# chenghuige/golden-huffman

Hardware: AMD Instinct MI355X
Metric: encode+decode GB/s (input bytes) (higher is better)
Workload: dtype u8

## Files before the change

golden-huffman_amd/csrc/ghf_internal.h:

```cpp
#ifndef GHF_INTERNAL_H_
#define GHF_INTERNAL_H_
#include <hip/hip_runtime.h>
#include <stdint.h>
#include <type_traits>
#include "ghf.h"

namespace ghf {

constexpr int kWave = 64;
constexpr int kSymPerLane = 16;
constexpr int kSymPerIter = kWave * kSymPerLane;
constexpr int kSegSymbols = 64;
constexpr int kBlockSymbols = 4096;
constexpr uint32_t kChunkQuantum = 4096;
constexpr uint32_t kMinChunk = 16384;
constexpr uint32_t kMaxChunk = 1u << 20;
constexpr uint32_t kEmitSlots = 256 * 3 * 8;

constexpr int kHistThreads = 256;
constexpr int kHistRep = 32;

constexpr int kEmitThreads = 512;
constexpr int kEmitWaves = kEmitThreads / kWave;
constexpr int kStageWords = 544;
constexpr int kStageCapBits = (kStageWords - 8) * 32;

constexpr int kDecPairBitsMax = 10;
constexpr int kDecLutBitsMax = 12;
constexpr int kDec7LutLog2 = 14;
constexpr int kDec7LutSlots = 1 << kDec7LutLog2;
constexpr int kDec7SmallSlots = 1024;

constexpr uint32_t kPlanesGroups = 256 * 16;
constexpr uint32_t kPlanesLdsBytes = 9 * 1024;
__host__ __device__ constexpr inline uint32_t planes_tile_elems(uint32_t elem_bytes) {
  return (uint32_t)kWave * (elem_bytes < 4 ? 4 : elem_bytes) * 16 / elem_bytes;
}
template <class F>
inline void with_elem_bytes(uint32_t elem_bytes, F&& f) {
  if (elem_bytes == 2) f(std::integral_constant<int, 2>());
  else if (elem_bytes == 4) f(std::integral_constant<int, 4>());
  else f(std::integral_constant<int, 8>());
}
constexpr int kPlanesHistThreads = 256;
constexpr int kPlanesHistCols = 32;
constexpr uint32_t kPlanesHistGroups = 256 * 4;
constexpr uint32_t kPlanesHistTileVecs = kPlanesHistThreads * 4;
constexpr uint32_t kPlanesHistFlushTiles = 3;
static_assert((uint64_t)(kPlanesHistFlushTiles + 1) * kPlanesHistTileVecs * 16 < (1ull << 32), "a u32 counter never wraps between two flushes");
constexpr size_t kPlanesHistAccWords = 32 * GHF_PLANES_MAX * 256;
constexpr uint32_t kSparseTile = 4096;
constexpr uint32_t kSparseGroups = 256 * 16;
constexpr uint32_t kSparseLdsBytes = 258 * 16;
constexpr size_t kSparseOffWords = kSparseGroups + 2;
constexpr uint32_t kSparseRankElems = 32768;
constexpr size_t kSparseRankHeaderBytes = 64;
constexpr uint64_t kSparseRankMagic = 0x314B4E4152464847ull;
constexpr uint32_t kSparseRankVersion = 1;
static_assert(kSparseRankElems == 8 * kBlockSymbols, "a rank block of the mask is one seek block");

constexpr uint64_t kHeaderFixedBytes = 4 * (GHF_NSYM + 3);
template <class T>
__host__ __device__ constexpr inline T header_bytes_for(T max_len) { return (T)kHeaderFixedBytes + 8 * max_len; }
__host__ __device__ constexpr inline uint64_t blocks_for(uint64_t n) { return (n + kBlockSymbols - 1) / kBlockSymbols; }
__host__ __device__ constexpr inline uint64_t segs_for(uint64_t n) { return (n + kSegSymbols - 1) / kSegSymbols; }
inline void index_shape(uint64_t n, ghf_index* ix) {
  ix->n_symbols = n;
  ix->chunk_symbols = kBlockSymbols;
  ix->seg_symbols = kSegSymbols;
  ix->n_chunks = blocks_for(n);
  ix->n_segs = segs_for(n);
}

inline uint32_t chunk_symbols_for(uint64_t n) {
  const uint64_t per_slot = (n + kEmitSlots - 1) / kEmitSlots;
  uint64_t c = (per_slot + kChunkQuantum - 1) / kChunkQuantum * kChunkQuantum;
  if (c < kMinChunk) c = kMinChunk;
  if (c > kMaxChunk) c = kMaxChunk;
  return (uint32_t)c;
}
inline uint64_t chunk_count_for(uint64_t n) {
  const uint64_t c = chunk_symbols_for(n);
  return (n + c - 1) / c;
}

struct DecTables {
  uint32_t fc_left[36];
  uint32_t start_pos[36];
  uint16_t symbol[GHF_NSYM + 3];
  int32_t min_len, max_len, lut_bits;
  int32_t pair_bits;
  int32_t kind;
  uint32_t root;
  uint16_t tl[256], tr[256];
  uint32_t ticket[16 * 32];
  uint32_t done;
  alignas(16) uint32_t image[kDec7LutSlots + kDec7SmallSlots];
};

struct EmitParams {
  const uint8_t* in;
  uint64_t n;
  const ghf_code* code;
  const uint64_t* chunk_off;
  const uint64_t* d_start_bit;
  uint8_t* out;
  uint64_t cap;
  uint32_t chunk;
  uint32_t nchunks;
  uint64_t* chunk_bit;
  uint32_t* seg_bit;
  int flags;
  int* status;
  uint64_t* d_end;
};

struct DecParams {
  const uint8_t* stream;
  uint64_t stream_bytes;
  DecTables* dt;
  const uint64_t* chunk_bit;
  const uint32_t* seg_bit;
  uint64_t n_symbols;
  uint64_t n_segs;
  uint32_t no_end_mark;
  uint8_t* out;
  uint64_t* out_bytes;
  int* status;
};

constexpr int kRunSymbols = 512;
constexpr int kRunsPerBlock = kBlockSymbols / kRunSymbols;
constexpr int kRunSegs = kRunSymbols / kSegSymbols;
constexpr size_t kSeekHeaderBytes = 64;
constexpr size_t kSeekRecordBytes = 24;
constexpr uint64_t kSeekMagic = 0x314B454553464847ull;
constexpr uint32_t kSeekVersion = 1;

struct SeekPackParams {
  const uint64_t* chunk_bit;
  const uint32_t* seg_bit;
  uint64_t n_symbols, n_blocks, n_segs;
  uint32_t flags;
  uint8_t* table;
  int* status;
};
struct SeekExpandParams {
  const uint8_t* records;
  const uint8_t* stream;
  uint64_t stream_bytes;
  const DecTables* dt;
  uint64_t n_symbols, n_blocks;
  uint64_t g0, g1;
  uint64_t* chunk_bit;
  uint32_t* seg_bit;
  int* status;
};
struct SeekExpandPlanesParams {
  SeekExpandParams plane[GHF_PLANES_MAX];
};
constexpr uint32_t kSeekStreamsMax = 2 * GHF_PLANES_MAX;
struct SeekExpandStreamsParams {
  SeekExpandParams stream[kSeekStreamsMax];
};
static_assert(sizeof(SeekExpandStreamsParams) <= 4096 - 64, "the parameter block stays under the kernel-argument limit");
struct DecHeadParams {
  const uint8_t* stream;
  uint64_t stream_bytes;
  const DecTables* dt;
  const uint64_t* chunk_bit;
  const uint32_t* seg_bit;
  uint64_t blk_sym0;
  uint64_t n_symbols;
  uint64_t lo, hi;
  uint8_t* out;
  int* status;
};

struct BatchCompressParams {
  const uint8_t* const* in_ptrs;
  const uint64_t* in_bytes;
  uint64_t max_item_bytes;
  uint8_t* const* out_ptrs;
  const uint64_t* out_caps;
  uint64_t* out_bytes;
  ghf_code* codes;
  uint64_t* chunk_bit;
  uint32_t* seg_bit;
  uint64_t blocks_per_item, segs_per_item;
  int* item_status;
};
struct BatchDecodeParams {
  const uint8_t* const* stream_ptrs;
  const uint64_t* stream_bytes;
  const ghf_code* codes;
  const uint64_t* chunk_bit;
  const uint32_t* seg_bit;
  uint64_t blocks_per_item, segs_per_item;
  uint64_t max_item_bytes;
  const uint64_t* n_symbols;
  uint8_t* const* out_ptrs;
  const uint64_t* out_caps;
  uint64_t* out_bytes;
  int* item_status;
};
struct BatchImagesParams {
  const uint8_t* const* stream_ptrs;
  const uint64_t* stream_bytes;
  uint64_t max_stream_bytes;
  uint8_t* const* out_ptrs;
  const uint64_t* out_caps;
  uint64_t* out_bytes;
  ghf_code* codes;
  int* item_status;
  uint64_t* stats;
};

struct BatchHistParams {
  const uint8_t* const* in_ptrs;
  const uint64_t* in_bytes;
  uint64_t max_item_bytes;
  uint32_t count;
  uint64_t* hist;
};
struct BatchSharedCompressParams {
  const uint8_t* const* in_ptrs;
  const uint64_t* in_bytes;
  uint64_t max_item_bytes;
  const ghf_code* code;
  uint8_t* const* out_ptrs;
  const uint64_t* out_caps;
  uint64_t* out_bytes;
  uint64_t* chunk_bit;
  uint32_t* seg_bit;
  uint64_t blocks_per_item, segs_per_item;
  int* item_status;
};
struct BatchSharedDecodeParams {
  const uint8_t* const* stream_ptrs;
  const uint64_t* stream_bytes;
  const ghf_code* code;
  const uint64_t* chunk_bit;
  const uint32_t* seg_bit;
  uint64_t blocks_per_item, segs_per_item;
  uint64_t max_item_bytes;
  const uint64_t* n_symbols;
  uint8_t* const* out_ptrs;
  const uint64_t* out_caps;
  uint64_t* out_bytes;
  int* item_status;
};
struct BatchSharedBodiesParams {
  const uint8_t* const* stream_ptrs;
  const uint64_t* stream_bytes;
  uint64_t max_stream_bytes;
  const ghf_code* code;
  uint8_t* const* out_ptrs;
  const uint64_t* out_caps;
  uint64_t* out_bytes;
  int* item_status;
  uint64_t* stats;
};

struct BatchPlanesHistParams {
  const uint8_t* const* in_ptrs;
  const uint64_t* in_bytes;
  uint64_t max_item_bytes;
  uint32_t count;
  uint64_t* hists;
};
struct BatchPlanesCompressParams {
  const uint8_t* const* in_ptrs;
  const uint64_t* in_bytes;
  uint64_t max_item_bytes;
  const ghf_code* codes;
  uint8_t* const* out_ptrs;
  const uint64_t* out_caps;
  uint64_t* out_bytes;
  uint64_t* chunk_bit;
  uint32_t* seg_bit;
  uint64_t blocks_per_item, segs_per_item;
  int* item_status;
};
struct BatchPlanesDecodeParams {
  const uint8_t* const* stream_ptrs;
  const uint64_t* stream_bytes;
  const ghf_code* codes;
  const uint64_t* chunk_bit;
  const uint32_t* seg_bit;
  uint64_t blocks_per_item, segs_per_item;
  uint64_t max_plane_symbols;
  const uint64_t* n_elems;
  uint8_t* const* out_ptrs;
  const uint64_t* out_caps;
  uint64_t* out_bytes;
  int* item_status;
};
struct BatchPlanesBodiesParams {
  const uint8_t* const* stream_ptrs;
  const uint64_t* stream_bytes;
  uint64_t max_stream_bytes;
  const ghf_code* codes;
  uint8_t* const* out_ptrs;
  const uint64_t* out_caps;
  uint64_t* out_bytes;
  int* item_status;
  uint64_t* stats;
};

constexpr uint32_t kBatchSeekMagic = 0x31524247u;
constexpr uint32_t kBatchRunSymbols = 128;
constexpr uint32_t kBatchRunSegs = kBatchRunSymbols / kSegSymbols;
constexpr uint32_t kBatchRunsPerBlock = kBlockSymbols / kBatchRunSymbols;
constexpr uint32_t kBatchSeekHeadBytes = 8;
__host__ __device__ constexpr inline uint64_t batch_runs_for(uint64_t n) { return (n + kBatchRunSymbols - 1) / kBatchRunSymbols; }
__host__ __device__ constexpr inline uint64_t batch_seek_bytes_for(uint64_t n) {
  return (kBatchSeekHeadBytes + 2 * batch_runs_for(n) + 7) & ~7ull;
}
struct BatchSeekPackParams {
  const uint64_t* chunk_bit;
  const uint32_t* seg_bit;
  uint64_t blocks_per_item, segs_per_item;
  uint64_t max_slice_symbols;
  const uint64_t* in_bytes;
  uint32_t elem_bytes;
  uint8_t* const* rec_ptrs;
  const uint64_t* rec_caps;
  uint64_t* rec_bytes;
  int* slot_status;
};
struct BatchSeekDecodeParams {
  const uint8_t* const* stream_ptrs;
  const uint64_t* stream_bytes;
  const uint8_t* const* rec_ptrs;
  const uint64_t* rec_bytes;
  uint64_t max_stream_bytes;
  const ghf_code* codes;
  uint8_t* const* out_ptrs;
  const uint64_t* out_caps;
  uint64_t* out_bytes;
  int* item_status;
};

enum SyncKind : uint32_t {
  kSyncCrs2 = 0,
  kSyncCrs = 1,
  kSyncPiece = 2,
};
struct SyncParams {
  const uint8_t* stream;
  uint64_t stream_bytes;
  uint64_t body_bit0;
  uint64_t end_bit;
  uint32_t no_eof;
  const DecTables* dt;
  uint64_t nsub;
  uint16_t* start;
  uint16_t* used;
  uint32_t* cnt;
  uint8_t* eof;
  uint32_t first;
  uint32_t first_start;
  uint32_t* changed;
  unsigned long long* moved_first_inv;
  uint64_t* eof_sub;
  uint64_t* tile_sum;
};

constexpr size_t kHistAccWords = 32 * 256 + 16 + 16 * 16;
void launch_histogram(const uint8_t* d_in, uint64_t n, uint32_t chunk, uint32_t nchunks, uint32_t* d_chunk_hist,
                      uint64_t* d_hist, uint64_t* d_acc, bool add, hipStream_t s);
void launch_build_code(const uint64_t* d_hist, ghf_code* d_code, int* d_status, uint32_t flags, hipStream_t s);
void launch_write_header(const ghf_code* d_code, uint8_t* d_out, uint64_t cap, int* d_status, hipStream_t s);
void launch_plan(const uint8_t* d_in, uint64_t n, uint32_t chunk, uint32_t nchunks, const uint32_t* d_chunk_hist,
                 const ghf_code* d_code, uint64_t* d_chunk_off, uint64_t* d_total_bits, hipStream_t s);
void launch_scan(uint64_t* d_v, uint32_t count, uint64_t* d_total, hipStream_t s);
void launch_crs_build_code(const uint64_t* d_hist, ghf_tree* d_tree, ghf_code* d_code, uint64_t* d_start_bit, int* d_status,
                           hipStream_t s);
void launch_crs_finish(const ghf_tree* d_tree, const uint64_t* d_total_bits, uint8_t* d_out, uint64_t* d_out_bytes, int* d_status,
                       hipStream_t s);
void launch_stream_copy(const uint8_t* d_src, uint8_t* d_dst, uint64_t n, bool nt, hipStream_t s);
void launch_store_u64(uint64_t* d_dst, const uint64_t* d_src_opt, uint64_t add, hipStream_t s);
void launch_load_u16(uint64_t* d_dst, const uint16_t* d_src, hipStream_t s);
void launch_shard_start(const ghf_code* d_code, const uint64_t* d_totals, int rank, uint64_t* d_start_bit, hipStream_t s);
void launch_emit(const EmitParams& p, hipStream_t s);
void launch_build_decode_tables(const ghf_code* d_code, DecTables* d_dt, int* d_status, hipStream_t s);
void launch_build_decode_tables_slots(const ghf_code* d_codes, DecTables* d_dts, uint32_t count, uint32_t slots, int* d_status, hipStream_t s);
void launch_crs_decode_tables(const ghf_tree* d_tree, DecTables* d_dt, int* d_status, hipStream_t s);
constexpr uint64_t kDecMaxGroups = 0xFFFF0000ull;
void launch_decode(const DecParams& p, hipStream_t s);
void launch_sync_pass(const SyncParams& p, hipStream_t s);
void launch_sync_counts(const SyncParams& p, uint64_t* d_total, hipStream_t s);
size_t sync_scan_workspace(uint64_t nsub);
void launch_sync_scan(const SyncParams& p, uint8_t* ws, uint32_t stride ,
                      uint32_t entry , hipStream_t s);
void launch_sync_index(const SyncParams& p, uint64_t* d_seg_abs, uint64_t n_symbols, uint64_t* d_chunk_bit, uint32_t* d_seg_bit,
                       hipStream_t s);
void launch_seek_pack(const SeekPackParams& p, hipStream_t s);
void launch_seek_expand(const SeekExpandParams& p, hipStream_t s);
void launch_seek_expand_planes(const SeekExpandPlanesParams& a, uint32_t planes, hipStream_t s);
void launch_seek_expand_streams(const SeekExpandStreamsParams& a, uint32_t streams, hipStream_t s);
void launch_decode_head(const DecHeadParams& p, hipStream_t s);
void launch_compress_batch(const BatchCompressParams& p, uint32_t count, hipStream_t s);
void launch_decode_batch(const BatchDecodeParams& p, uint32_t count, hipStream_t s);
void launch_decode_images_batch(const BatchImagesParams& p, uint32_t count, hipStream_t s);
void launch_histogram_batch(const BatchHistParams& p, uint32_t flags, hipStream_t s);
void launch_compress_batch_shared(const BatchSharedCompressParams& p, uint32_t count, hipStream_t s);
void launch_decode_batch_shared(const BatchSharedDecodeParams& p, uint32_t count, hipStream_t s);
void launch_decode_bodies_batch_shared(const BatchSharedBodiesParams& p, uint32_t count, hipStream_t s);
void launch_histogram_batch_finish(uint64_t* d_hists, uint32_t n_hists, uint32_t flags, hipStream_t s);
void launch_histogram_batch_planes(const BatchPlanesHistParams& p, uint32_t elem_bytes, uint32_t flags, hipStream_t s);
void launch_build_codes(const uint64_t* d_hists, uint32_t n_codes, ghf_code* d_codes, int* d_status, uint32_t flags, hipStream_t s);
void launch_batch_planes_raw_auto(const uint64_t* d_hists, const ghf_code* d_codes, uint32_t elem_bytes, uint32_t* d_raw_planes,
                                  hipStream_t s);
void launch_compress_batch_planes(const BatchPlanesCompressParams& p, uint32_t count, uint32_t elem_bytes, bool forms, uint32_t raw_planes,
                                  hipStream_t s);
void launch_decode_batch_planes(const BatchPlanesDecodeParams& p, uint32_t count, uint32_t elem_bytes, bool forms, uint32_t raw_planes,
                                hipStream_t s);
void launch_decode_bodies_batch_planes(const BatchPlanesBodiesParams& p, uint32_t count, uint32_t elem_bytes, bool forms,
                                       uint32_t raw_planes, hipStream_t s);
void launch_batch_seek_pack(const BatchSeekPackParams& p, uint32_t slots, hipStream_t s);
void launch_decode_bodies_batch_seek(const BatchSeekDecodeParams& p, uint32_t count, uint32_t elem_bytes, bool forms, uint32_t raw_planes,
                                     hipStream_t s);
void launch_planes_split(const uint8_t* d_in, const uint8_t* d_base, uint64_t n_elems, uint32_t elem_bytes, uint8_t* d_planes,
                         uint64_t plane_stride, hipStream_t s);
void launch_planes_merge(const uint8_t* d_planes, uint64_t plane_stride, const uint8_t* d_base, uint64_t n_elems, uint32_t elem_bytes,
                         uint8_t* d_out, const int* d_status, hipStream_t s);
void launch_planes_merge_range(const uint8_t* d_planes, uint64_t plane_stride, const uint8_t* d_base, uint64_t first, uint64_t count,
                               uint32_t elem_bytes, uint8_t* d_out, const int* d_status, hipStream_t s);
void launch_planes_split_to(const uint8_t* d_in, const uint8_t* d_base, uint64_t n_elems, uint32_t elem_bytes, uint8_t* const* h_dst,
                            hipStream_t s);
void launch_planes_merge_from(const uint8_t* const* h_src, const uint8_t* d_base, uint64_t n_elems, uint32_t elem_bytes, uint8_t* d_out,
                              const int* d_status, hipStream_t s);
void launch_sparse_split(const uint8_t* d_in, uint64_t n, uint8_t* d_mask, uint8_t* d_vals, uint64_t vals_cap, uint64_t* d_n_vals,
                         uint64_t* d_counts, uint64_t* d_offs, int* d_status, hipStream_t s);
void launch_sparse_merge(const uint8_t* d_mask, const uint8_t* d_vals, uint64_t n_vals, uint64_t n, uint8_t* d_out, uint64_t* d_counts,
                         uint64_t* d_offs, int* d_status, hipStream_t s);
void launch_sparse_merge_at(const uint8_t* d_mask, const uint8_t* d_vals, uint64_t vals_skip, uint64_t n_vals, uint64_t n, uint8_t* d_out,
                            uint64_t* d_counts, uint64_t* d_offs, int* d_status, hipStream_t s);
void launch_sparse_rank_pack(const uint8_t* d_mask, uint64_t n, uint8_t* d_table, uint64_t* d_counts, uint64_t* d_offs, int* d_status,
                             hipStream_t s);
hipError_t launch_histogram_planes(const uint8_t* d_in, const uint8_t* d_base, uint64_t n_elems, uint32_t elem_bytes, uint32_t flags,
                                   uint64_t* d_acc, uint64_t* d_hists, hipStream_t s);
void launch_planes_image_bytes(const uint64_t* d_hists, const ghf_code* d_codes, uint32_t elem_bytes, uint64_t* d_bytes, hipStream_t s);
void launch_planes_vet_codes(const uint64_t* d_hists, const ghf_code* d_codes, uint32_t elem_bytes, int* d_status, hipStream_t s);

struct PlanesGatherParams {
  const uint8_t* streams[GHF_PLANES_MAX];
  uint64_t stream_bytes[GHF_PLANES_MAX];
  const uint8_t* records[GHF_PLANES_MAX];
  const ghf_code* codes;
  uint64_t n_elems, n_blocks;
  const uint64_t* index;
  uint64_t index_stride;
  uint32_t row_elems, n_rows;
  uint32_t stage_bytes;
  uint8_t* out;
  uint64_t out_stride;
  int32_t* row_status;
};
void launch_decode_planes_gather(const PlanesGatherParams& p, uint32_t elem_bytes, uint32_t raw_planes, hipStream_t s);

struct PlanesGatherFormsParams {
  const uint8_t* streams[2 * GHF_PLANES_MAX];
  uint64_t stream_bytes[2 * GHF_PLANES_MAX];
  const uint8_t* records[2 * GHF_PLANES_MAX];
  const uint64_t* cum[GHF_PLANES_MAX];
  uint64_t n_vals[GHF_PLANES_MAX];
  const ghf_code* codes;
  const uint8_t* base;
  uint64_t n_elems;
  const uint64_t* index;
  uint64_t index_stride;
  uint32_t row_elems, n_rows;
  uint32_t stage_bytes;
  uint32_t once;
  uint8_t* out;
  uint64_t out_stride;
  int32_t* row_status;
};
void launch_decode_planes_gather_forms(const PlanesGatherFormsParams& p, uint32_t elem_bytes, uint32_t raw_planes, uint32_t sparse_planes,
                                       hipStream_t s);

}
#endif
```

golden-huffman_amd/csrc/ghf_kernels.hip:

```cpp
#include "ghf_build_code.h"

namespace ghf {

#define GHF_HADD(x, sh) atomicAdd(&lh[((((x) >> (sh)) & 0xFFu) << 5) | rep], 1u)

__device__ __forceinline__ void hist_vec(uint32_t* lh, uint32_t rep, const uint4& v) {
  GHF_HADD(v.x, 0); GHF_HADD(v.x, 8); GHF_HADD(v.x, 16); GHF_HADD(v.x, 24);
  GHF_HADD(v.y, 0); GHF_HADD(v.y, 8); GHF_HADD(v.y, 16); GHF_HADD(v.y, 24);
  GHF_HADD(v.z, 0); GHF_HADD(v.z, 8); GHF_HADD(v.z, 16); GHF_HADD(v.z, 24);
  GHF_HADD(v.w, 0); GHF_HADD(v.w, 8); GHF_HADD(v.w, 16); GHF_HADD(v.w, 24);
}

__global__ __launch_bounds__(kHistThreads) void k_histogram(const uint8_t* __restrict__ in, uint64_t n,
                                                            uint32_t chunk32, uint32_t nchunks,
                                                            uint32_t* __restrict__ chunk_hist,
                                                            unsigned long long* __restrict__ hist,
                                                            unsigned long long* __restrict__ acc ,
                                                            uint32_t add ) {
  static_assert(kHistRep == 32, "replica index is lane % 32");
  __shared__ uint32_t lh[256 * kHistRep];
  __shared__ bool s_last;
  const uint32_t tid = threadIdx.x;
  const uint32_t rep = tid & 31u;
  uint32_t prev = 0;
  unsigned long long total = 0;
  const uint64_t chunk = chunk32;
  const uint32_t V = chunk32 >> 12;
  const uint32_t nfullchunks = (uint32_t)(n / chunk);
  const bool fast = V >= 4u && (chunk32 & 4095u) == 0 && (((uintptr_t)in) & 15u) == 0 && nfullchunks > 0;
  auto vptr = [&](uint32_t c, uint32_t j) -> const uint4* {
    if (c >= nfullchunks) c = nfullchunks - 1;
    return reinterpret_cast<const uint4*>(in + (uint64_t)c * chunk) + (uint64_t)j * kHistThreads + tid;
  };
  uint4 A = make_uint4(0, 0, 0, 0), B = A;
  if (fast) {
    A = load_stream(vptr(blockIdx.x, 0));
    B = load_stream(vptr(blockIdx.x, 1));
  }
  for (uint32_t i = tid; i < 256 * kHistRep; i += kHistThreads) lh[i] = 0;
  __syncthreads();

  __shared__ uint32_t s_tick;
  auto finish_chunk = [&](uint32_t c) -> uint32_t {
    __syncthreads();
    const uint32_t posted = s_tick;
    uint32_t s = 0;
#pragma unroll
    for (uint32_t j = 0; j < kHistRep; ++j) s += lh[(tid << 5) | ((j + tid) & 31u)];
    const uint32_t cnt = s - prev;
    prev = s;
    chunk_hist[(uint64_t)c * 256 + tid] = cnt;
    total += cnt;
    __syncthreads();
    return posted;
  };

  if (fast) {
    const uint32_t ncls = gridDim.x < 16u ? 1u : (gridDim.x < 128u ? gridDim.x >> 3 : 16u);
    const uint32_t cls = (blockIdx.x >> 3) % ncls;
    unsigned long long* tick = acc + 32 * 256 + 16 + cls * 16;
    auto draw = [&]() -> uint32_t { return 2u * gridDim.x + (uint32_t)atomicAdd(tick, 1ull) * ncls + cls; };
    uint32_t cur = blockIdx.x;
    uint32_t nxt = blockIdx.x + gridDim.x;
    auto vat = [&](uint32_t g) -> const uint4* { return g < V ? vptr(cur, g) : vptr(nxt, g - V); };
    const uint32_t Vmain = V & ~3u, Vrest = V & 3u;
    while (cur < nfullchunks) {
      uint32_t t_next = 0;
      if (tid == 0) t_next = draw();
      for (uint32_t j = 0; j < Vmain; j += 4) {
        const uint4 C = load_stream(vat(j + 2)), D = load_stream(vat(j + 3));
        hist_vec(lh, rep, A);
        hist_vec(lh, rep, B);
        A = load_stream(vat(j + 4));
        B = load_stream(vat(j + 5));
        hist_vec(lh, rep, C);
        hist_vec(lh, rep, D);
      }
      if (Vrest == 1u) {
        hist_vec(lh, rep, A);
        A = B;
        B = load_stream(vptr(nxt, 1));
      } else if (Vrest == 2u) {
        hist_vec(lh, rep, A);
        hist_vec(lh, rep, B);
        A = load_stream(vptr(nxt, 0));
        B = load_stream(vptr(nxt, 1));
      } else if (Vrest == 3u) {
        const uint4 C = load_stream(vptr(cur, V - 1));
        hist_vec(lh, rep, A);
        hist_vec(lh, rep, B);
        A = load_stream(vptr(nxt, 0));
        B = load_stream(vptr(nxt, 1));
        hist_vec(lh, rep, C);
      }
      if (tid == 0) s_tick = t_next;
      const uint32_t posted = finish_chunk(cur);
      cur = nxt;
      nxt = posted;
    }
  }

  const uint32_t g0 = fast ? (blockIdx.x == 0 ? nfullchunks : nchunks) : blockIdx.x;
  const uint32_t gstep = fast ? nchunks : gridDim.x;
  for (uint32_t c = g0; c < nchunks; c += gstep) {
    const uint64_t base = (uint64_t)c * chunk;
    const uint64_t len = (n - base < chunk) ? (n - base) : chunk;
    const uint8_t* p = in + base;
    uint32_t head = (uint32_t)((16u - (uint32_t)((uintptr_t)p & 15u)) & 15u);
    if (head > len) head = (uint32_t)len;
    if (tid < head) atomicAdd(&lh[((uint32_t)p[tid] << 5) | rep], 1u);
    const uint4* pv = reinterpret_cast<const uint4*>(p + head);
    const uint64_t nvec = (len - head) >> 4;
    for (uint64_t i = tid; i < nvec; i += kHistThreads) {
      const uint4 v0 = pv[i];
      hist_vec(lh, rep, v0);
    }
    const uint64_t tail0 = head + (nvec << 4);
    if (tail0 + tid < len) atomicAdd(&lh[((uint32_t)p[tail0 + tid] << 5) | rep], 1u);
    (void)finish_chunk(c);
  }
  unsigned long long* rep_base = acc + (uint64_t)(blockIdx.x & 31u) * 256;
  if (total) atomicAdd(&rep_base[tid], total);
  asm volatile("s_waitcnt vmcnt(0)" ::: "memory");
  __syncthreads();
  if (tid == 0) {
    const unsigned long long t = atomicAdd(&acc[32 * 256], 1ull);
    s_last = (t + 1 == gridDim.x);
    if (s_last) __builtin_amdgcn_fence(__ATOMIC_ACQUIRE, "agent");
    asm volatile("s_waitcnt vmcnt(0)" ::: "memory");
  }
  __syncthreads();
  if (s_last) {
    unsigned long long part[32];
#pragma unroll
    for (int r = 0; r < 32; ++r) part[r] = __hip_atomic_load(&acc[r * 256 + tid], __ATOMIC_RELAXED, __HIP_MEMORY_SCOPE_AGENT);
    unsigned long long sum = 0;
#pragma unroll
    for (int r = 0; r < 32; ++r) {
      sum += part[r];
      __hip_atomic_store(&acc[r * 256 + tid], 0ull, __ATOMIC_RELAXED, __HIP_MEMORY_SCOPE_AGENT);
    }
    hist[tid] = add ? hist[tid] + sum : sum;
    if (tid < 16) __hip_atomic_store(&acc[32 * 256 + 16 + tid * 16], 0ull, __ATOMIC_RELAXED, __HIP_MEMORY_SCOPE_AGENT);
    if (tid == 0) {
      hist[256] = 1;
      __hip_atomic_store(&acc[32 * 256], 0ull, __ATOMIC_RELAXED, __HIP_MEMORY_SCOPE_AGENT);
    }
  }
}

void launch_histogram(const uint8_t* d_in, uint64_t n, uint32_t chunk, uint32_t nchunks, uint32_t* d_chunk_hist,
                      uint64_t* d_hist, uint64_t* d_acc, bool add, hipStream_t s) {
  static int ncu = 0;
  if (ncu == 0) {
    int dev = 0;
    hipDeviceProp_t prop;
    if (hipGetDevice(&dev) == hipSuccess && hipGetDeviceProperties(&prop, dev) == hipSuccess) ncu = prop.multiProcessorCount;
    if (ncu < 1) ncu = 256;
  }
  uint32_t grid = (uint32_t)(4 * ncu);
  if (grid > nchunks) grid = nchunks;
  if (grid == 0) grid = 1;
  hipLaunchKernelGGL(k_histogram, dim3(grid), dim3(kHistThreads), 0, s, d_in, n, chunk, nchunks, d_chunk_hist,
                     reinterpret_cast<unsigned long long*>(d_hist), reinterpret_cast<unsigned long long*>(d_acc),
                     add ? 1u : 0u);
}

template <bool LIMIT>
__global__ __launch_bounds__(64) void k_build_code(const unsigned long long* __restrict__ hist, ghf_code* __restrict__ out,
                                                   int* __restrict__ status, uint32_t empty_ok) {
  __shared__ HeapLds heap;
  __shared__ typename std::conditional<LIMIT, LimitLds, NoLimitLds>::type Q;
  __builtin_amdgcn_s_setprio(3);
  __shared__ CodeLds cl;
  __shared__ int s_ndata;
  build_code_body<LIMIT, true>(heap, Q, cl, s_ndata, HistCounts{hist}, out, status, empty_ok, threadIdx.x);
}

void launch_build_code(const uint64_t* d_hist, ghf_code* d_code, int* d_status, uint32_t flags, hipStream_t s) {
  if (flags & GHF_CODE_LIMIT)
    hipLaunchKernelGGL(k_build_code<true>, dim3(1), dim3(64), 0, s, reinterpret_cast<const unsigned long long*>(d_hist), d_code, d_status,
                       flags & GHF_EMPTY_OK);
  else
    hipLaunchKernelGGL(k_build_code<false>, dim3(1), dim3(64), 0, s, reinterpret_cast<const unsigned long long*>(d_hist), d_code, d_status,
                       flags & GHF_EMPTY_OK);
}

struct TreeLds {
  uint16_t tl[256], tr[256];
  uint16_t size[GHF_NSYM + 256 + 7];
  uint8_t is_right[GHF_NSYM + 256 + 7];
  uint32_t code_hi[256];
  uint32_t max_len, min_len;
  int n;
};

__global__ __launch_bounds__(64) void k_crs_build_code(const unsigned long long* __restrict__ hist, ghf_tree* __restrict__ out_tree,
                                                       ghf_code* __restrict__ out_code, unsigned long long* __restrict__ start_bit,
                                                       int* __restrict__ status) {
  __shared__ HeapLds heap;
  __shared__ TreeLds T;
  __shared__ ghf_tree tree;
  __builtin_amdgcn_s_setprio(3);
  const int lane = threadIdx.x;
  {
    u64t mine = 0;
    bool any_big = false;
#pragma unroll
    for (int j = 0; j < 4; ++j) {
      const u64t f = hist[lane + 64 * j];
      mine += f;
      any_big |= (f >> GHF_HIST_TOTAL_BITS) != 0;
    }
    if (counts_out_of_domain(mine, any_big)) {
      if (lane == 0) latch_status(status, GHF_E_INVAL);
      return;
    }
  }
  for (int s = lane; s < GHF_NSYM; s += 64) heap.cur[s] = (uint16_t)s;
  for (int i = lane; i < GHF_NSYM + 256 + 7; i += 64) {
    heap.parent[i] = 0;
    T.size[i] = 1;
    T.is_right[i] = 0;
  }
  for (int i = lane; i < (int)(sizeof(ghf_tree) / 4); i += 64) reinterpret_cast<uint32_t*>(&tree)[i] = 0;
  if (lane == 0) {
    T.max_len = 0;
    T.min_len = 0xFFFFFFFFu;
  }
  __syncthreads();
  int n = 0;
  for (int s = 0; s < 256; ++s) {
    const u64t f = wave_uniform((u64t)hist[s]);
    if (f) {
      wave_heap_push(heap, n, (f << 9) | (u64t)s, lane);
      ++n;
    }
  }
  const int nleaves = n;
  if (nleaves < 2) {
    if (lane == 0) latch_status(status, nleaves == 0 ? GHF_E_EMPTY : GHF_E_SINGLE);
    return;
  }
  const int times = n - 1;
  for (int t = 0; t < times; ++t) {
    const u64t e1 = wave_heap_pop(heap, n, lane);
    const u64t e2 = wave_heap_pop(heap, n, lane);
    const int s1 = (int)(e1 & 511u), s2 = (int)(e2 & 511u);
    const int node = GHF_NSYM + t;
    if (lane == 0) {
      const int a = heap.cur[s1], b = heap.cur[s2];
      heap.parent[a] = (uint16_t)node;
      heap.parent[b] = (uint16_t)node;
      T.tl[t] = (uint16_t)a;
      T.tr[t] = (uint16_t)b;
      T.is_right[b] = 1;
      T.size[node] = (uint16_t)(1 + T.size[a] + T.size[b]);
      heap.cur[s2] = (uint16_t)node;
    }
    wave_heap_push(heap, n, (((e1 >> 9) + (e2 >> 9)) << 9) | (u64t)s2, lane);
    ++n;
  }
  __syncthreads();
  for (int v = lane; v < GHF_NSYM + times; v += 64) {
    const bool leaf = v < 256;
    if (v == 256 || (leaf && heap.parent[v] == 0)) continue;
    uint32_t len = 0, pre = 0;
    unsigned long long code = 0;
    int x = v;
    for (int p; (p = heap.parent[x]) != 0; x = p) {
      const uint32_t r = T.is_right[x];
      if (len < 64) code |= (unsigned long long)r << len;
      ++len;
      pre += 1u + (r ? (uint32_t)T.size[T.tl[p - GHF_NSYM]] : 0u);
    }
    if (leaf) {
      tree.header[2 * pre] = 0;
      tree.header[2 * pre + 1] = (uint8_t)v;
      atomicMax(&T.max_len, len);
      atomicMin(&T.min_len, len);
      if (len <= 64) {
        out_code->length[v] = len;
        out_code->codeword[v] = (uint32_t)code;
        T.code_hi[v] = (uint32_t)(code >> 32);
      }
    } else {
      tree.header[2 * pre] = 255;
      tree.header[2 * pre + 1] = 255;
      const int t = v - GHF_NSYM;
      const int a = T.tl[t], b = T.tr[t];
      tree.left[t] = (uint16_t)(a < GHF_NSYM ? a : 256 + (a - GHF_NSYM));
      tree.right[t] = (uint16_t)(b < GHF_NSYM ? b : 256 + (b - GHF_NSYM));
    }
  }
  __syncthreads();
  const bool deep = T.max_len > 32u;
  for (int s = lane; s < GHF_NSYM; s += 64) {
    const bool absent = s == 256 || heap.parent[s] == 0;
    if (absent) {
      out_code->length[s] = 0;
      out_code->codeword[s] = 0;
    }
    out_code->symbol[s] = deep ? (absent ? 0u : T.code_hi[s]) : 0xFFFFFFFFu;
  }
  for (int i = lane; i < 64; i += 64) {
    out_code->first_code[i] = 0;
    out_code->start_pos[i] = 0;
  }
  if (T.max_len > 64u) {
    if (lane == 0) latch_status(status, GHF_E_CODELEN);
    return;
  }
  if (lane == 0) {
    tree.root = (uint32_t)(256 + times - 1);
    tree.n_leaves = (uint32_t)nleaves;
    tree.max_len = T.max_len;
    tree.tree_bytes = 2u * (2u * (uint32_t)nleaves - 1u);
    out_code->min_len = (int32_t)T.min_len;
    out_code->max_len = (int32_t)T.max_len;
    if (start_bit) *start_bit = 8ull * ((unsigned long long)tree.tree_bytes + 2ull);
  }
  __syncthreads();
  for (int i = lane; i < (int)(sizeof(ghf_tree) / 4); i += 64)
    reinterpret_cast<uint32_t*>(out_tree)[i] = reinterpret_cast<const uint32_t*>(&tree)[i];
}

void launch_crs_build_code(const uint64_t* d_hist, ghf_tree* d_tree, ghf_code* d_code, uint64_t* d_start_bit, int* d_status,
                           hipStream_t s) {
  hipLaunchKernelGGL(k_crs_build_code, dim3(1), dim3(64), 0, s, reinterpret_cast<const unsigned long long*>(d_hist), d_tree,
                     d_code, reinterpret_cast<unsigned long long*>(d_start_bit), d_status);
}

__global__ __launch_bounds__(256) void k_crs_finish(const ghf_tree* __restrict__ tree, const unsigned long long* __restrict__ total_bits,
                                                    uint8_t* __restrict__ out, unsigned long long* __restrict__ out_bytes,
                                                    const int* __restrict__ status) {
  if (*status != 0) return;
  const uint32_t tb = tree->tree_bytes;
  for (uint32_t i = threadIdx.x; i < tb; i += 256) out[i] = tree->header[i];
  if (threadIdx.x == 0) {
    const unsigned long long t = *total_bits;
    const unsigned long long whole = t >> 3;
    const uint32_t left = (uint32_t)((8u - (uint32_t)(t & 7u)) & 7u);
    out[tb] = (uint8_t)left;
    out[tb + 1] = left ? out[tb + 2 + whole] : (uint8_t)0;
    if (out_bytes) *out_bytes = (unsigned long long)tb + 2ull + whole;
  }
}

void launch_crs_finish(const ghf_tree* d_tree, const uint64_t* d_total_bits, uint8_t* d_out, uint64_t* d_out_bytes, int* d_status,
                       hipStream_t s) {
  hipLaunchKernelGGL(k_crs_finish, dim3(1), dim3(256), 0, s, d_tree, reinterpret_cast<const unsigned long long*>(d_total_bits), d_out,
                     reinterpret_cast<unsigned long long*>(d_out_bytes), d_status);
}

__global__ __launch_bounds__(256) void k_write_header(const ghf_code* __restrict__ code, uint8_t* __restrict__ out,
                                                      uint64_t cap, int* __restrict__ status) {
  const int max_len = code->max_len;
  if (max_len < 1 || max_len > 32) return;
  const int nwords = 1 + GHF_NSYM + 2 + 2 * max_len;
  if ((uint64_t)nwords * 4 > cap) {
    if (threadIdx.x == 0) latch_status(status, GHF_E_CAP);
    return;
  }
  uint32_t* o = reinterpret_cast<uint32_t*>(out);
  for (int w = threadIdx.x; w < nwords; w += blockDim.x) o[w] = bswap32(header_word(code, w, max_len));
}

void launch_write_header(const ghf_code* d_code, uint8_t* d_out, uint64_t cap, int* d_status, hipStream_t s) {
  hipLaunchKernelGGL(k_write_header, dim3(1), dim3(256), 0, s, d_code, d_out, cap, d_status);
}

__global__ __launch_bounds__(256) void k_chunk_bits(const uint32_t* __restrict__ chunk_hist, uint32_t nchunks,
                                                    const ghf_code* __restrict__ code, uint64_t* __restrict__ bits) {
  const int lane = threadIdx.x & 63;
  const uint32_t wave = (blockIdx.x * blockDim.x + threadIdx.x) >> 6;
  const uint32_t nwaves = (gridDim.x * blockDim.x) >> 6;
  const uint4 L = reinterpret_cast<const uint4*>(code->length)[lane];
  for (uint32_t c = wave; c < nchunks; c += nwaves) {
    const uint4 h = reinterpret_cast<const uint4*>(chunk_hist + (uint64_t)c * 256)[lane];
    unsigned long long b = (unsigned long long)h.x * L.x + (unsigned long long)h.y * L.y +
                           (unsigned long long)h.z * L.z + (unsigned long long)h.w * L.w;
#pragma unroll
    for (int d = 32; d >= 1; d >>= 1) b += __shfl_xor(b, d, 64);
    if (lane == 0) bits[c] = b;
  }
}

__global__ __launch_bounds__(256) void k_chunk_bits_direct(const uint8_t* __restrict__ in, uint64_t n, uint32_t chunk32,
                                                           uint32_t nchunks, const ghf_code* __restrict__ code,
                                                           uint64_t* __restrict__ bits) {
  __shared__ uint32_t ll[256];
  ll[threadIdx.x] = code->length[threadIdx.x];
  __syncthreads();
  const int lane = threadIdx.x & 63;
  const uint32_t wave = (blockIdx.x * blockDim.x + threadIdx.x) >> 6;
  const uint32_t nwaves = (gridDim.x * blockDim.x) >> 6;
  const uint64_t chunk = chunk32;
  for (uint32_t c = wave; c < nchunks; c += nwaves) {
    const uint64_t base = (uint64_t)c * chunk;
    const uint64_t len = (n - base < chunk) ? (n - base) : chunk;
    unsigned long long b = 0;
    const uint8_t* p = in + base;
    uint64_t head = (16u - (uint32_t)((uintptr_t)p & 15u)) & 15u;
    if (head > len) head = len;
    if ((uint64_t)lane < head) b += ll[p[lane]];
    const uint4* pv = reinterpret_cast<const uint4*>(p + head);
    const uint64_t nvec = (len - head) >> 4;
    uint32_t acc = 0;
    for (uint64_t i = lane; i < nvec; i += 64) {
      const uint4 v = pv[i];
      const uint32_t w[4] = {v.x, v.y, v.z, v.w};
#pragma unroll
      for (int k = 0; k < 4; ++k)
        acc += ll[w[k] & 0xFFu] + ll[(w[k] >> 8) & 0xFFu] + ll[(w[k] >> 16) & 0xFFu] + ll[w[k] >> 24];
      if ((i >> 6) % 4096u == 4095u) {
        b += acc;
        acc = 0;
      }
    }
    b += acc;
    const uint64_t tail0 = head + (nvec << 4);
    if (tail0 + (uint64_t)lane < len) b += ll[p[tail0 + lane]];
#pragma unroll
    for (int d = 32; d >= 1; d >>= 1) b += __shfl_xor(b, d, 64);
    if (lane == 0) bits[c] = b;
  }
}

__global__ __launch_bounds__(1024) void k_scan(uint64_t* __restrict__ v, uint32_t count, uint64_t* __restrict__ total_out) {
  __shared__ unsigned long long wsum[16];
  const int tid = threadIdx.x, lane = tid & 63, w = tid >> 6;
  const uint32_t ipt = (count + 1023u) / 1024u;
  const uint32_t lo = tid * ipt;
  const uint32_t hi = (lo + ipt < count) ? lo + ipt : count;
  unsigned long long mine = 0;
  const bool small = ipt <= 8u;
  unsigned long long x8[8];
  if (small) {
#pragma unroll
    for (uint32_t k = 0; k < 8; ++k) {
      const uint32_t i = lo + k;
      x8[k] = (k < ipt && i < hi) ? v[i] : 0ull;
    }
#pragma unroll
    for (uint32_t k = 0; k < 8; ++k) mine += x8[k];
  } else {
    for (uint32_t i = lo; i < hi; ++i) mine += v[i];
  }
  unsigned long long s = mine;
#pragma unroll
  for (int d = 1; d < 64; d <<= 1) {
    const unsigned long long t = __shfl_up(s, d, 64);
    if (lane >= d) s += t;
  }
  if (lane == 63) wsum[w] = s;
  __syncthreads();
  unsigned long long woff = 0, total = 0;
  for (int k = 0; k < 16; ++k) {
    const unsigned long long x = wsum[k];
    if (k < w) woff += x;
    total += x;
  }
  unsigned long long run = woff + s - mine;
  if (small) {
#pragma unroll
    for (uint32_t k = 0; k < 8; ++k) {
      const uint32_t i = lo + k;
      if (k < ipt && i < hi) v[i] = run;
      run += x8[k];
    }
  } else {
    for (uint32_t i = lo; i < hi; ++i) {
      const unsigned long long x = v[i];
      v[i] = run;
      run += x;
    }
  }
  if (tid == 0) {
    v[count] = total;
    if (total_out) *total_out = total;
  }
}

void launch_scan(uint64_t* d_v, uint32_t count, uint64_t* d_total, hipStream_t s) {
  hipLaunchKernelGGL(k_scan, dim3(1), dim3(1024), 0, s, d_v, count, d_total);
}

void launch_plan(const uint8_t* d_in, uint64_t n, uint32_t chunk, uint32_t nchunks, const uint32_t* d_chunk_hist,
                 const ghf_code* d_code, uint64_t* d_chunk_off, uint64_t* d_total_bits, hipStream_t s) {
  uint32_t blocks = (nchunks + 3) / 4;
  if (blocks > 2048) blocks = 2048;
  if (blocks == 0) blocks = 1;
  if (d_chunk_hist)
    hipLaunchKernelGGL(k_chunk_bits, dim3(blocks), dim3(256), 0, s, d_chunk_hist, nchunks, d_code, d_chunk_off);
  else
    hipLaunchKernelGGL(k_chunk_bits_direct, dim3(blocks), dim3(256), 0, s, d_in, n, chunk, nchunks, d_code,
                       d_chunk_off);
  hipLaunchKernelGGL(k_scan, dim3(1), dim3(1024), 0, s, d_chunk_off, nchunks, d_total_bits);
}

__global__ void k_store_u64(uint64_t* dst, const uint64_t* src, uint64_t add) { *dst = (src ? *src : 0ull) + add; }
void launch_store_u64(uint64_t* d_dst, const uint64_t* d_src_opt, uint64_t add, hipStream_t s) {
  hipLaunchKernelGGL(k_store_u64, dim3(1), dim3(1), 0, s, d_dst, d_src_opt, add);
}

__global__ void k_load_u16(uint64_t* dst, const uint16_t* src) { *dst = *src; }
void launch_load_u16(uint64_t* d_dst, const uint16_t* d_src, hipStream_t s) { hipLaunchKernelGGL(k_load_u16, dim3(1), dim3(1), 0, s, d_dst, d_src); }

__global__ void k_shard_start(const ghf_code* code, const uint64_t* totals, int rank, uint64_t* start_bit) {
  uint64_t b = 8ull * header_bytes_for((uint64_t)code->max_len);
  for (int r = 0; r < rank; ++r) b += totals[r];
  *start_bit = b;
}
void launch_shard_start(const ghf_code* d_code, const uint64_t* d_totals, int rank, uint64_t* d_start_bit, hipStream_t s) {
  hipLaunchKernelGGL(k_shard_start, dim3(1), dim3(1), 0, s, d_code, d_totals, rank, d_start_bit);
}

template <bool NT>
__global__ __launch_bounds__(256) void k_stream_copy(const uint4* __restrict__ src, uint4* __restrict__ dst, uint64_t nvec) {
  const uint64_t per = (nvec + gridDim.x - 1) / gridDim.x;
  const uint64_t lo = (uint64_t)blockIdx.x * per;
  const uint64_t end = lo + per < nvec ? lo + per : nvec;
  uint64_t i = lo + threadIdx.x;
  auto ld = [&](uint64_t k) -> uint4 { return NT ? load_stream(src + k) : src[k]; };
  auto st = [&](uint64_t k, const uint4& v) {
    if (NT) store_stream(dst + k, v);
    else dst[k] = v;
  };
  for (; i + 3 * 256 < end; i += 4 * 256) {
    const uint4 a = ld(i), b = ld(i + 256), c = ld(i + 512), d = ld(i + 768);
    st(i, a); st(i + 256, b); st(i + 512, c); st(i + 768, d);
  }
  for (; i < end; i += 256) st(i, ld(i));
}
__global__ void k_tail_copy(const uint8_t* src, uint8_t* dst, uint64_t from, uint64_t n) {
  const uint64_t i = from + threadIdx.x;
  if (i < n) dst[i] = src[i];
}
void launch_stream_copy(const uint8_t* d_src, uint8_t* d_dst, uint64_t n, bool nt, hipStream_t s) {
  const uint64_t nvec = n / 16;
  if (nvec) {
    uint64_t blocks = (nvec + 255) / 256;
    if (blocks > 4096) blocks = 4096;
    if (nt) hipLaunchKernelGGL(k_stream_copy<true>, dim3((uint32_t)blocks), dim3(256), 0, s, reinterpret_cast<const uint4*>(d_src), reinterpret_cast<uint4*>(d_dst), nvec);
    else hipLaunchKernelGGL(k_stream_copy<false>, dim3((uint32_t)blocks), dim3(256), 0, s, reinterpret_cast<const uint4*>(d_src), reinterpret_cast<uint4*>(d_dst), nvec);
  }
  if (n & 15) hipLaunchKernelGGL(k_tail_copy, dim3(1), dim3(16), 0, s, d_src, d_dst, nvec * 16, n);
}

}
```

Measured before the change: 952.9.

## Double-buffer histogram LDS sets across 512-thread blocks with deeper prefetch

The histogram kernel moves to 512 threads split into two halves that alternate chunk rows. It keeps two LDS replica sets, so one half can reduce and store the finished chunk while both halves keep counting the next chunk, and it drops one of the two barriers per chunk. Five stream loads are kept in flight across chunk boundaries, using a three-deep queue of chunk indices. The final last-block detection becomes a two-level counter per class, and the grid is halved to keep occupancy. The cost is more LDS per block and more complex control flow in the kernel's ticket scheduling.

Result: no change. 960.5 (median of 6 runs) (+0.8%).

```diff
diff --git a/golden-huffman_amd/csrc/ghf_internal.h b/golden-huffman_amd/csrc/ghf_internal.h
--- a/golden-huffman_amd/csrc/ghf_internal.h
+++ b/golden-huffman_amd/csrc/ghf_internal.h
@@ -17,7 +17,7 @@
 constexpr uint32_t kMaxChunk = 1u << 20;
 constexpr uint32_t kEmitSlots = 256 * 3 * 8;
 
-constexpr int kHistThreads = 256;
+constexpr int kHistThreads = 512;
 constexpr int kHistRep = 32;
 
 constexpr int kEmitThreads = 512;
diff --git a/golden-huffman_amd/csrc/ghf_kernels.hip b/golden-huffman_amd/csrc/ghf_kernels.hip
--- a/golden-huffman_amd/csrc/ghf_kernels.hip
+++ b/golden-huffman_amd/csrc/ghf_kernels.hip
@@ -18,119 +18,140 @@
                                                             unsigned long long* __restrict__ acc ,
                                                             uint32_t add ) {
   static_assert(kHistRep == 32, "replica index is lane % 32");
-  __shared__ uint32_t lh[256 * kHistRep];
+  static_assert(kHistThreads == 512, "two halves of 256 threads: one thread of a half per bin");
+  constexpr uint32_t kSetWords = 256 * kHistRep;
+  __shared__ uint32_t lh[2 * kSetWords];
+  __shared__ uint32_t s_tick[2];
   __shared__ bool s_last;
   const uint32_t tid = threadIdx.x;
   const uint32_t rep = tid & 31u;
+  const uint32_t bin = tid & 255u;
+  const uint32_t half = (uint32_t)__builtin_amdgcn_readfirstlane((int)(tid >> 8));
   uint32_t prev = 0;
   unsigned long long total = 0;
+  uint32_t k = 0;
   const uint64_t chunk = chunk32;
   const uint32_t V = chunk32 >> 12;
   const uint32_t nfullchunks = (uint32_t)(n / chunk);
   const bool fast = V >= 4u && (chunk32 & 4095u) == 0 && (((uintptr_t)in) & 15u) == 0 && nfullchunks > 0;
-  auto vptr = [&](uint32_t c, uint32_t j) -> const uint4* {
+  auto vptr = [&](uint32_t c, uint32_t row) __attribute__((always_inline)) -> const uint4* {
     if (c >= nfullchunks) c = nfullchunks - 1;
-    return reinterpret_cast<const uint4*>(in + (uint64_t)c * chunk) + (uint64_t)j * kHistThreads + tid;
+    return reinterpret_cast<const uint4*>(in + (uint64_t)c * chunk) + (uint64_t)row * 256 + bin;
   };
-  uint4 A = make_uint4(0, 0, 0, 0), B = A;
+  auto rows_of = [&](uint32_t s) __attribute__((always_inline)) -> uint32_t { return (V + 1u - (half ^ (s & 1u))) >> 1; };
+
+  const uint32_t ncls = gridDim.x < 16u ? 1u : (gridDim.x < 128u ? gridDim.x >> 3 : 16u);
+  const uint32_t cls = (blockIdx.x >> 3) % ncls;
+  unsigned long long* tick = acc + 32 * 256 + 16 + cls * 16;
+  auto draw = [&]() __attribute__((always_inline)) -> uint32_t { return atomicAdd(reinterpret_cast<uint32_t*>(tick), 1u); };
+  auto drawn_chunk = [&](uint32_t t) __attribute__((always_inline)) -> uint32_t { return 3u * gridDim.x + t * ncls + cls; };
+  uint32_t cur = blockIdx.x, qa = cur + gridDim.x, qb = qa + gridDim.x;
+  uint32_t l_ahead = 0, l_row = half, l_left = rows_of(0);
+#define GHF_K1_ISSUE(R)                                                            \
+  do {                                                                             \
+    if (l_left == 0) {                                                             \
+      ++l_ahead;                                                                   \
+      l_row = half ^ ((k + l_ahead) & 1u);                                         \
+      l_left = rows_of(k + l_ahead);                                               \
+    }                                                                              \
+    const uint32_t l_chunk = l_ahead == 0 ? cur : (l_ahead == 1u ? qa : qb);       \
+    R = load_stream(vptr(l_chunk, l_row));                                         \
+    l_row += 2;                                                                    \
+    --l_left;                                                                      \
+  } while (0)
+  uint4 R0 = make_uint4(0, 0, 0, 0), R1 = R0, R2 = R0, R3 = R0, R4 = R0;
   if (fast) {
-    A = load_stream(vptr(blockIdx.x, 0));
-    B = load_stream(vptr(blockIdx.x, 1));
-  }
-  for (uint32_t i = tid; i < 256 * kHistRep; i += kHistThreads) lh[i] = 0;
-  __syncthreads();
-
-  __shared__ uint32_t s_tick;
-  auto finish_chunk = [&](uint32_t c) -> uint32_t {
-    __syncthreads();
-    const uint32_t posted = s_tick;
+    GHF_K1_ISSUE(R0); GHF_K1_ISSUE(R1); GHF_K1_ISSUE(R2); GHF_K1_ISSUE(R3); GHF_K1_ISSUE(R4);
+  }
+  for (uint32_t i = tid; i < 2 * kSetWords / 4; i += kHistThreads) reinterpret_cast<uint4*>(lh)[i] = make_uint4(0, 0, 0, 0);
+  __syncthreads();
+
+  auto reduce_store = [&](const uint32_t* set, uint32_t c) __attribute__((always_inline)) {
     uint32_t s = 0;
 #pragma unroll
-    for (uint32_t j = 0; j < kHistRep; ++j) s += lh[(tid << 5) | ((j + tid) & 31u)];
+    for (uint32_t j = 0; j < kHistRep; ++j) s += set[(bin << 5) | ((j + bin) & 31u)];
     const uint32_t cnt = s - prev;
     prev = s;
-    chunk_hist[(uint64_t)c * 256 + tid] = cnt;
+    chunk_hist[(uint64_t)c * 256 + bin] = cnt;
     total += cnt;
-    __syncthreads();
-    return posted;
   };
 
-  if (fast) {
-    const uint32_t ncls = gridDim.x < 16u ? 1u : (gridDim.x < 128u ? gridDim.x >> 3 : 16u);
-    const uint32_t cls = (blockIdx.x >> 3) % ncls;
-    unsigned long long* tick = acc + 32 * 256 + 16 + cls * 16;
-    auto draw = [&]() -> uint32_t { return 2u * gridDim.x + (uint32_t)atomicAdd(tick, 1ull) * ncls + cls; };
-    uint32_t cur = blockIdx.x;
-    uint32_t nxt = blockIdx.x + gridDim.x;
-    auto vat = [&](uint32_t g) -> const uint4* { return g < V ? vptr(cur, g) : vptr(nxt, g - V); };
-    const uint32_t Vmain = V & ~3u, Vrest = V & 3u;
-    while (cur < nfullchunks) {
-      uint32_t t_next = 0;
-      if (tid == 0) t_next = draw();
-      for (uint32_t j = 0; j < Vmain; j += 4) {
-        const uint4 C = load_stream(vat(j + 2)), D = load_stream(vat(j + 3));
-        hist_vec(lh, rep, A);
-        hist_vec(lh, rep, B);
-        A = load_stream(vat(j + 4));
-        B = load_stream(vat(j + 5));
-        hist_vec(lh, rep, C);
-        hist_vec(lh, rep, D);
-      }
-      if (Vrest == 1u) {
-        hist_vec(lh, rep, A);
-        A = B;
-        B = load_stream(vptr(nxt, 1));
-      } else if (Vrest == 2u) {
-        hist_vec(lh, rep, A);
-        hist_vec(lh, rep, B);
-        A = load_stream(vptr(nxt, 0));
-        B = load_stream(vptr(nxt, 1));
-      } else if (Vrest == 3u) {
-        const uint4 C = load_stream(vptr(cur, V - 1));
-        hist_vec(lh, rep, A);
-        hist_vec(lh, rep, B);
-        A = load_stream(vptr(nxt, 0));
-        B = load_stream(vptr(nxt, 1));
-        hist_vec(lh, rep, C);
-      }
-      if (tid == 0) s_tick = t_next;
-      const uint32_t posted = finish_chunk(cur);
-      cur = nxt;
-      nxt = posted;
-    }
+  if (fast && cur < nfullchunks) {
+    uint32_t* set = lh;
+    uint32_t left = rows_of(0);
+    uint32_t t_next = 0;
+    if (tid == 0) t_next = draw();
+    bool over = false;
+#define GHF_K1_STEP(R)                                                                              \
+  {                                                                                                 \
+    if (!over) {                                                                                    \
+      hist_vec(set, rep, R);                                                                        \
+      if (--left == 0) {                                                                            \
+        if (tid == 0) s_tick[k & 1u] = drawn_chunk(t_next);                                         \
+        __syncthreads();                                                                            \
+        const uint32_t posted = (uint32_t)__builtin_amdgcn_readfirstlane((int)s_tick[k & 1u]);      \
+        if (half == (k & 1u)) reduce_store(set, cur);                                               \
+        ++k;                                                                                        \
+        --l_ahead;                \
+        cur = qa;                                                                                   \
+        qa = qb;                                                                                    \
+        qb = posted;                                                                                \
+        over = cur >= nfullchunks;                                                                  \
+        set = lh + (k & 1u) * kSetWords;                                                            \
+        left = rows_of(k);                                                                          \
+        if (tid == 0) t_next = draw();               \
+      }                                                                                             \
+    }                                                                                               \
+    GHF_K1_ISSUE(R);                                                                                \
+  }
+    do {
+      GHF_K1_STEP(R0)
+      GHF_K1_STEP(R1)
+      GHF_K1_STEP(R2)
+      GHF_K1_STEP(R3)
+      GHF_K1_STEP(R4)
+    } while (!over);
+#undef GHF_K1_STEP
+#undef GHF_K1_ISSUE
   }
 
   const uint32_t g0 = fast ? (blockIdx.x == 0 ? nfullchunks : nchunks) : blockIdx.x;
   const uint32_t gstep = fast ? nchunks : gridDim.x;
   for (uint32_t c = g0; c < nchunks; c += gstep) {
+    uint32_t* set = lh + (k & 1u) * kSetWords;
     const uint64_t base = (uint64_t)c * chunk;
     const uint64_t len = (n - base < chunk) ? (n - base) : chunk;
     const uint8_t* p = in + base;
     uint32_t head = (uint32_t)((16u - (uint32_t)((uintptr_t)p & 15u)) & 15u);
     if (head > len) head = (uint32_t)len;
-    if (tid < head) atomicAdd(&lh[((uint32_t)p[tid] << 5) | rep], 1u);
+    if (tid < head) atomicAdd(&set[((uint32_t)p[tid] << 5) | rep], 1u);
     const uint4* pv = reinterpret_cast<const uint4*>(p + head);
     const uint64_t nvec = (len - head) >> 4;
     for (uint64_t i = tid; i < nvec; i += kHistThreads) {
       const uint4 v0 = pv[i];
-      hist_vec(lh, rep, v0);
+      hist_vec(set, rep, v0);
     }
     const uint64_t tail0 = head + (nvec << 4);
-    if (tail0 + tid < len) atomicAdd(&lh[((uint32_t)p[tail0 + tid] << 5) | rep], 1u);
-    (void)finish_chunk(c);
+    if (tail0 + tid < len) atomicAdd(&set[((uint32_t)p[tail0 + tid] << 5) | rep], 1u);
+    __syncthreads();
+    if (half == (k & 1u)) reduce_store(set, c);
+    ++k;
   }
   unsigned long long* rep_base = acc + (uint64_t)(blockIdx.x & 31u) * 256;
-  if (total) atomicAdd(&rep_base[tid], total);
+  if (total) atomicAdd(&rep_base[bin], total);
   asm volatile("s_waitcnt vmcnt(0)" ::: "memory");
   __syncthreads();
   if (tid == 0) {
-    const unsigned long long t = atomicAdd(&acc[32 * 256], 1ull);
-    s_last = (t + 1 == gridDim.x);
-    if (s_last) __builtin_amdgcn_fence(__ATOMIC_ACQUIRE, "agent");
+    const uint32_t groups = gridDim.x >> 3;
+    const uint32_t in_cls = 8u * (groups / ncls + (cls < groups % ncls ? 1u : 0u)) + (groups % ncls == cls ? (gridDim.x & 7u) : 0u);
+    bool last = false;
+    if (atomicAdd(tick + 1, 1ull) + 1 == in_cls) last = atomicAdd(&acc[32 * 256], 1ull) + 1 == ncls;
+    s_last = last;
+    if (last) __builtin_amdgcn_fence(__ATOMIC_ACQUIRE, "agent");
     asm volatile("s_waitcnt vmcnt(0)" ::: "memory");
   }
   __syncthreads();
-  if (s_last) {
+  if (s_last && tid < 256) {
     unsigned long long part[32];
 #pragma unroll
     for (int r = 0; r < 32; ++r) part[r] = __hip_atomic_load(&acc[r * 256 + tid], __ATOMIC_RELAXED, __HIP_MEMORY_SCOPE_AGENT);
@@ -141,7 +162,8 @@
       __hip_atomic_store(&acc[r * 256 + tid], 0ull, __ATOMIC_RELAXED, __HIP_MEMORY_SCOPE_AGENT);
     }
     hist[tid] = add ? hist[tid] + sum : sum;
-    if (tid < 16) __hip_atomic_store(&acc[32 * 256 + 16 + tid * 16], 0ull, __ATOMIC_RELAXED, __HIP_MEMORY_SCOPE_AGENT);
+    if (tid < 32)
+      __hip_atomic_store(&acc[32 * 256 + 16 + (tid >> 1) * 16 + (tid & 1u)], 0ull, __ATOMIC_RELAXED, __HIP_MEMORY_SCOPE_AGENT);
     if (tid == 0) {
       hist[256] = 1;
       __hip_atomic_store(&acc[32 * 256], 0ull, __ATOMIC_RELAXED, __HIP_MEMORY_SCOPE_AGENT);
@@ -158,7 +180,7 @@
     if (hipGetDevice(&dev) == hipSuccess && hipGetDeviceProperties(&prop, dev) == hipSuccess) ncu = prop.multiProcessorCount;
     if (ncu < 1) ncu = 256;
   }
-  uint32_t grid = (uint32_t)(4 * ncu);
+  uint32_t grid = (uint32_t)(2 * ncu);
   if (grid > nchunks) grid = nchunks;
   if (grid == 0) grid = 1;
   hipLaunchKernelGGL(k_histogram, dim3(grid), dim3(kHistThreads), 0, s, d_in, n, chunk, nchunks, d_chunk_hist,
```
